# graphdeco-inria/editable-gaussian-reflections

Hardware: AMD Instinct MI355X
Metric: Mrays/s fwd+bwd @1080p, 1M Gaussians (higher is better)
Workload: dtype f32; 1 GPU; BASELINE config C: synthetic dense-init room+spheres cloud, HEADLINE variant = init (literal dense-init opacity 0.1 (config.py:44): Kc ~ 22 per ray, bounces mostly die), N=1000000, 1920x1080, one training iteration: export + update_bvh + forward + backward + grad import, num_bounces=2, jitter on, reference default config; variant=init, gaussians=1000000, width=1920, height=1080, parallelism=image tiles x1 + 1 all-reduce of the launch's [22N] gradients, team_help=product default (on)

## Files before the change

### editable-gaussian-reflections_amd/csrc/forward_task.inc

```
        const uint32_t task = tq;
        const TaskGeom tg = task_geom(v, tb, lane);
        const StateRef S = state_of(v, task, lane);
        const size_t chain_head = (size_t)step * (BATCH ? v.num_tasks * v.batch_frames : v.num_tasks) + task;
        if (GRADS && lane == 0) v.task_last_block[chain_head] = 0xFFFFFFFFu;
        if constexpr (OBJ) {
            for (uint32_t j = 0; j < oq.num_bits; j++) oacc[j * EGR_WAVE + (uint32_t)lane] = 0.0f;
        }

        bool active = tg.inside;
        f3 ro = mk3(0, 0, 0), rd = mk3(0, 0, 1);
        uint32_t seed = 0;
        if (step == 0) {
            if (active) {
                if constexpr (BATCH) {
                    seed = tea4(tg.pixel_id, (uint32_t)*v.meta.total_num_calls + bframe + 1u);
                    ro = mk3(bcam[0], bcam[1], bcam[2]);
                    rd = primary_direction(v, tg.px, tg.py, *v.cfg.jitter_primary_rays != 0, seed, bcam[12], bcam + 3);
                } else {
                    seed = tea4(tg.pixel_id, (uint32_t)*v.meta.total_num_calls);
                    ro = mk3(v.cam.origin[0], v.cam.origin[1], v.cam.origin[2]);
                    rd = primary_direction(v, tg.px, tg.py, *v.cfg.jitter_primary_rays != 0, seed, tanf(*v.cam.vertical_fov_radians / 2.0f), v.cam.rotation_w2c);
                }
            }
        } else {
// ... 22 lines not shown
            return e < v.ext_blocks_cap ? e : EGR_EXT_NONE - 1u;
        };
        double full_Td = 1.0;
        float full_T = 1.0f;
        bool overflow = false;
        EGR_STATS(uint32_t st_visits = 0, st_leafhits = 0, st_inner = 0, st_outer = 0, st_batches = 0u; unsigned long long st_eval_cycles = 0ull, st_batch_cycles = 0ull;)
        int seg = 0;
        float seg_lo, seg_hi;
        auto evaluate = [&](uint32_t prim, const float4 &w0, const float4 &w1, const float4 &w2, auto a2src, const f3 &lo_pre) {
            float t = 0.0f, alpha = 0.0f;
            const int r = test_candidate<CUBE, false>(fc, step, seg, near_plane, ro, rd, prim, w0, w1, w2, a2src, t, alpha, &lo_pre);
            if (r == 0 || r == 3) return;
            traversed++;
            if (r == 1) return;
            full_Td *= 1.0 - (double)alpha;
            if (cnt < v.cand_cap) {
                keys[EGR_KEY_AT(lane, cnt)] = t;
                vals[EGR_VAL_AT(lane, cnt)] = make_float2(alpha, u2f(prim));
                cnt++;
            } else {
                if (ext == EGR_EXT_NONE) ext = ext_alloc();
                const uint32_t e = cnt - v.cand_cap;
                if (ext < EGR_EXT_NONE - 1u && e < EGR_EXT_BLOCK) {
                    v.ext_keys[(size_t)ext * EGR_EXT_BLOCK + e] = t;
                    v.ext_vals[(size_t)ext * EGR_EXT_BLOCK + e] = make_float2(alpha, u2f(prim));
                    cnt++;
                } else {
                    overflow = true;
                }
            }
        };
        const bool packet = step == 0 && v.rays_per_task == (uint32_t)EGR_WAVE;
        const bool by_pairs = !packet;
        if (by_pairs) {
            rayp[lane][0] = make_float4(ro.x, ro.y, ro.z, rd.x), rayp[lane][1] = make_float4(rd.y, rd.z, invq.x, invq.y), rayp[lane][2] = make_float4(invq.z, ncq.x, ncq.y, ncq.z);
            gcnt[lane] = 0u, gtrav[lane] = 0u, gext[lane] = EGR_EXT_NONE;
        }
        bool beyond_far_empty = false;
        if (!sentinels) {
            const float fx0 = v.frame.ox - 2.0f / v.frame.sx, fx1 = v.frame.ox + 65534.0f / v.frame.sx;
            const float fy0 = v.frame.oy - 2.0f / v.frame.sy, fy1 = v.frame.oy + 65534.0f / v.frame.sy;
            const float fz0 = v.frame.oz - 2.0f / v.frame.sz, fz1 = v.frame.oz + 65534.0f / v.frame.sz;
            const float dx = fmaxf(fabsf(ro.x - fx0), fabsf(ro.x - fx1)), dy = fmaxf(fabsf(ro.y - fy0), fabsf(ro.y - fy1)),
                        dz = fmaxf(fabsf(ro.z - fz0), fabsf(ro.z - fz1));
            const bool reaches = !(dx * dx + dy * dy + dz * dz < far_plane * far_plane * 0.999f);
            beyond_far_empty = __ballot(ray_ok && reaches) == 0ull;
        }
        const float near_c = near_plane, far_c = far_plane;
        seg_lo = near_c, seg_hi = far_c;
        for (seg = 0; seg < (CUBE ? 1 : 3); seg++) {
            if (seg == 1) {
                if (!(near_plane > 0.0f)) continue;
                seg_lo = 0.0f, seg_hi = near_c;
            } else if (seg == 2) {
                if (beyond_far_empty) continue;
                seg_lo = far_c, seg_hi = 3.0e38f;
            }
        if (packet) {
            const unsigned long long okm = __ballot(ray_ok);
            if (okm != 0ull) {
                auto wsum = [](float x) {
#pragma unroll
                    for (int off = 32; off > 0; off >>= 1) x += __shfl_xor(x, off);
                    return x;
                };
                auto wmin = [](float x) {
#pragma unroll
                    for (int off = 32; off > 0; off >>= 1) x = fminf(x, __shfl_xor(x, off));
                    return x;
                };
                auto wmax = [](float x) {
#pragma unroll
                    for (int off = 32; off > 0; off >>= 1) x = fmaxf(x, __shfl_xor(x, off));
                    return x;
                };
                auto uni = [](float x) { return u2f((uint32_t)__builtin_amdgcn_readfirstlane((int)f2u(x))); };
                const f3 dz = ray_ok ? rd : mk3(0, 0, 0);
                const f3 ew = normalize(mk3(wsum(dz.x), wsum(dz.y), wsum(dz.z)));
                const f3 eu = normalize(cross(fabsf(ew.z) < 0.9f ? mk3(0, 0, 1) : mk3(1, 0, 0), ew)), ev = cross(ew, eu);
                const float pw = dot(rd, ew), pu = dot(rd, eu) / pw, pv = dot(rd, ev) / pw;
                const bool narrow = wmin(ray_ok ? pw : 1.0f) > 0.5f && isfinite(ew.x + ew.y + ew.z);
                const float big = 3.0e38f, lat = 4e-6f;
                const float umin = narrow ? fminf(wmin(ray_ok ? pu : big) - lat, -lat) : -big, umax = narrow ? fmaxf(wmax(ray_ok ? pu : -big) + lat, lat) : big;
                const float vmin = narrow ? fminf(wmin(ray_ok ? pv : big) - lat, -lat) : -big, vmax = narrow ? fmaxf(wmax(ray_ok ? pv : -big) + lat, lat) : big;
                const float kappa = narrow ? wmax(ray_ok ? 1.0f / pw : 1.0f) * 1.000001f : big;
                const float isx = 1.0f / v.frame.sx, isy = 1.0f / v.frame.sy, isz = 1.0f / v.frame.sz;
                const f3 cam_o = BATCH ? mk3(bcam[0], bcam[1], bcam[2]) : mk3(v.cam.origin[0], v.cam.origin[1], v.cam.origin[2]);
                const float oqx = (cam_o.x - v.frame.ox) * v.frame.sx + 2.0f, oqy = (cam_o.y - v.frame.oy) * v.frame.sy + 2.0f, oqz = (cam_o.z - v.frame.oz) * v.frame.sz + 2.0f;
                const float hux = uni(0.5f * eu.x * isx), huy = uni(0.5f * eu.y * isy), huz = uni(0.5f * eu.z * isz);
                const float hvx = uni(0.5f * ev.x * isx), hvy = uni(0.5f * ev.y * isy), hvz = uni(0.5f * ev.z * isz);
                const float hwx = uni(0.5f * ew.x * isx), hwy = uni(0.5f * ew.y * isy), hwz = uni(0.5f * ew.z * isz);
                const float cu = uni(2.0f * (hux * oqx + huy * oqy + huz * oqz)), cv = uni(2.0f * (hvx * oqx + hvy * oqy + hvz * oqz)), cw = uni(2.0f * (hwx * oqx + hwy * oqy + hwz * oqz));
                const float slack = uni(isx + isy + isz);
                const float f_umin = uni(umin), f_umax = uni(umax), f_vmin = uni(vmin), f_vmax = uni(vmax), f_kappa = uni(kappa);
                const float f_lo = uni(seg_lo), f_hi = uni(seg_hi);
                const bool narrow_u = __builtin_amdgcn_readfirstlane(narrow ? 1 : 0) != 0;
                auto frustum_hit = [&](const uint4 &q) -> bool {
                    const float lx = (float)(q.x & 0xFFFFu), ly = (float)(q.x >> 16), lz = (float)(q.y & 0xFFFFu);
                    const float hx = (float)(q.y >> 16), hy = (float)(q.z & 0xFFFFu), hz = (float)(q.z >> 16);
                    const float cx = lx + hx, cy = ly + hy, cz = lz + hz, ex = hx - lx, ey = hy - ly, ez = hz - lz;
                    const float u1 = fmaf(hux, cx, fmaf(huy, cy, fmaf(huz, cz, -cu))), u2 = fmaf(fabsf(hux), ex, fmaf(fabsf(huy), ey, fabsf(huz) * ez));
                    const float v1 = fmaf(hvx, cx, fmaf(hvy, cy, fmaf(hvz, cz, -cv))), v2 = fmaf(fabsf(hvx), ex, fmaf(fabsf(hvy), ey, fabsf(hvz) * ez));
                    const float w1 = fmaf(hwx, cx, fmaf(hwy, cy, fmaf(hwz, cz, -cw))), w2 = fmaf(fabsf(hwx), ex, fmaf(fabsf(hwy), ey, fabsf(hwz) * ez));
                    const float wmx = w1 + w2 + slack, wmn = w1 - w2 - slack;
                    bool keep = wmx > 0.0f;
                    if (!narrow_u) return true;
                    keep &= fmaf(-f_umin, wmx, u1 + u2) >= -slack;
                    keep &= fmaf(f_umax, wmx, u2 - u1) >= -slack;
                    keep &= fmaf(-f_vmin, wmx, v1 + v2) >= -slack;
                    keep &= fmaf(f_vmax, wmx, v2 - v1) >= -slack;
                    keep &= wmx * f_kappa >= f_lo;
                    keep &= wmn <= f_hi;
                    if (sentinels) keep |= ((q.x & 0xFFFFu) == 0u) | ((q.x >> 16) == 0u) | ((q.y & 0xFFFFu) == 0u) | ((q.y >> 16) == 65535u) | ((q.z & 0xFFFFu) == 65535u) | ((q.z >> 16) == 65535u);
                    return keep;
                };
                const float n_umin = sqrtf(fmaf(f_umin, f_umin, 1.0f)), n_umax = sqrtf(fmaf(f_umax, f_umax, 1.0f)), n_vmin = sqrtf(fmaf(f_vmin, f_vmin, 1.0f)), n_vmax = sqrtf(fmaf(f_vmax, f_vmax, 1.0f));
                const uint32_t m = (uint32_t)lane & 7u, grp = (uint32_t)lane >> 3;
                uint32_t *__restrict__ ugstk = v.stack_spill + (size_t)slot * EGR_GSTK * EGR_WAVE;
                constexpr uint32_t UGSTK_CAP = (uint32_t)EGR_GSTK * EGR_WAVE;
                bool f_over = false;
                uint32_t top = 1u, nl = 0u;
                if (lane == 0) pstk[0] = 0u;
                wave_sync();
                for (;;) {
                    const bool do_eval = nl >= (uint32_t)EGR_WAVE || (top == 0u && nl > 0u);
                    if (!do_eval && top == 0u) break;
                    if (do_eval) {
                        EGR_STATS(const unsigned long long te0 = __builtin_amdgcn_s_memtime();)
                        if (narrow_u) {
                            EGR_STATS(const unsigned long long tf0 = __builtin_amdgcn_s_memtime(); st_batches += nl;)
                            uint32_t nk = 0u;
                            for (uint32_t base = 0u; base < nl; base += (uint32_t)EGR_WAVE) {
                                const uint32_t nb = min(nl - base, (uint32_t)EGR_WAVE);
                                const uint32_t leaf = lbuf[base + min((uint32_t)lane, nb - 1u)];
                                const float4 sp = v.bsph[leaf];
                                const f3 a = mk3(sp.x - cam_o.x, sp.y - cam_o.y, sp.z - cam_o.z);
                                const float au = dot(a, eu), av = dot(a, ev), aw = dot(a, ew);
                                const float rad = sqrtf(fmaxf(sp.w, 0.0f)) * 1.005f + 2e-6f * (fabsf(a.x) + fabsf(a.y) + fabsf(a.z));
                                bool keep = (uint32_t)lane < nb && sp.w >= 0.0f;
                                keep = keep && !(fmaf(f_umin, aw, -au) > rad * n_umin) && !(fmaf(-f_umax, aw, au) > rad * n_umax);
                                keep = keep && !(fmaf(f_vmin, aw, -av) > rad * n_vmin) && !(fmaf(-f_vmax, aw, av) > rad * n_vmax);
                                wave_sync();
                                const unsigned long long km = __builtin_amdgcn_ballot_w64(keep);
                                if (keep) lbuf[nk + __builtin_amdgcn_mbcnt_hi((uint32_t)(km >> 32), __builtin_amdgcn_mbcnt_lo((uint32_t)km, 0u))] = leaf;
                                nk += (uint32_t)__popcll(km);
                                wave_sync();
                            }
                            nl = nk;
                            EGR_STATS(st_batch_cycles += __builtin_amdgcn_s_memtime() - tf0;)
                        }
                        EGR_TIMES_IS(9, chain_leaves += nl;)
                        if (nl != 0u) {
                        static_assert(EGR_WAVE + 8 * EGR_FPOP * EGR_WIDTH <= 3 * EGR_WAVE, "the ray table holds one float4 per buffered leaf");
                        float4 *const llo = &rayp[0][0];
                        for (uint32_t base = 0u; base < nl; base += (uint32_t)EGR_WAVE) {
                            const uint32_t li = base + (uint32_t)lane;
                            if (li < nl) {
                                const uint32_t leaf = lbuf[li];
                                const float4 g0 = v.inst_w[4 * (size_t)leaf], g1 = v.inst_w[4 * (size_t)leaf + 1], g2 = v.inst_w[4 * (size_t)leaf + 2];
                                const f3 lo_ = object_origin(g0, g1, g2, cam_o);
                                llo[li] = make_float4(lo_.x, lo_.y, lo_.z, 0.0f);
                            }
                        }
                        wave_sync();
                        uint32_t pn = (uint32_t)__builtin_amdgcn_readfirstlane((int)lbuf[0]);
                        float4 n0 = load_f4_uniform(v.inst_w, 4 * pn), n1 = load_f4_uniform(v.inst_w, 4 * pn + 1), n2 = load_f4_uniform(v.inst_w, 4 * pn + 2), n3 = load_f4_uniform(v.inst_w, 4 * pn + 3);
                        uint32_t pn_next = lbuf[min(1u, nl - 1u)];
                        float4 nlo = llo[0];
#pragma unroll 1
                        for (uint32_t i = 0; i < nl; i++) {
                            const uint32_t p = pn;
                            const float4 w0 = n0, w1 = n1, w2 = n2, a2 = n3;
                            const f3 lo_pre = mk3(nlo.x, nlo.y, nlo.z);
                            pn = (uint32_t)__builtin_amdgcn_readfirstlane((int)pn_next);
                            pn_next = lbuf[min(i + 2u, nl - 1u)];
                            n0 = load_f4_uniform(v.inst_w, 4 * pn), n1 = load_f4_uniform(v.inst_w, 4 * pn + 1), n2 = load_f4_uniform(v.inst_w, 4 * pn + 2), n3 = load_f4_uniform(v.inst_w, 4 * pn + 3);
                            nlo = llo[min(i + 1u, nl - 1u)];
                            EGR_STATS(st_leafhits += ray_ok ? 1u : 0u, st_outer += (lane == 0);)
                            if (ray_ok) evaluate(p, w0, w1, w2, a2, lo_pre);
#if defined(__HIP_DEVICE_COMPILE__)
                            asm volatile("" ::"s"(n0.w), "s"(n1.w), "s"(n2.w), "s"(n3.x), "s"(n3.y));
#endif
                        }
                        }
                        nl = 0u;
                        wave_sync();
                        EGR_STATS(st_eval_cycles += __builtin_amdgcn_s_memtime() - te0;)
                        if (top == 0u) break;
                    }
                    const uint32_t npop = min(top, 8u * (uint32_t)EGR_FPOP);
                    uint4 sl_[EGR_FPOP];
#pragma unroll
                    for (int u = 0; u < EGR_FPOP; u++) {
                        const uint32_t gi = grp + 8u * (uint32_t)u;
                        const uint32_t e = top - 1u - min(gi, top - 1u);
                        uint32_t node = pstk[min(e, (uint32_t)EGR_PSTK - 1u)];
                        if (top > (uint32_t)EGR_PSTK && e >= (uint32_t)EGR_PSTK) node = __hip_atomic_load(ugstk + (e - EGR_PSTK), __ATOMIC_RELAXED, __HIP_MEMORY_SCOPE_AGENT);
                        sl_[u] = wnodes[(size_t)node * EGR_WIDTH + m];
                        if (!(gi < npop)) sl_[u].w = EGR_EMPTY_SLOT;
                        EGR_STATS(st_visits += (m == 0u && gi < npop) ? 1u : 0u;)
                    }
                    top -= npop;
                    EGR_STATS(st_inner += (lane == 0);)
                    wave_sync();
#pragma unroll
                    for (int u = 0; u < EGR_FPOP; u++) {
                        const uint4 sl = sl_[u];
                        const bool hit = frustum_hit(sl) & (sl.w != EGR_EMPTY_SLOT);
                        const bool leaf = (int)sl.w < 0;
                        const unsigned long long hm = __builtin_amdgcn_ballot_w64(hit), lm = __builtin_amdgcn_ballot_w64(leaf);
                        const unsigned long long im = hm & ~lm, fm = hm & lm;
                        const uint32_t at = top + __builtin_amdgcn_mbcnt_hi((uint32_t)(im >> 32), __builtin_amdgcn_mbcnt_lo((uint32_t)im, 0u));
                        if (hit & !leaf) {
                            if (at < (uint32_t)EGR_PSTK) pstk[at] = sl.w;
                            else if (at - EGR_PSTK < UGSTK_CAP) __hip_atomic_store(ugstk + (at - EGR_PSTK), sl.w, __ATOMIC_RELAXED, __HIP_MEMORY_SCOPE_AGENT);
                            else f_over = true;
                        }
                        top = min(top + (uint32_t)__popcll(im), (uint32_t)EGR_PSTK + UGSTK_CAP);
                        if (hit & leaf) lbuf[nl + __builtin_amdgcn_mbcnt_hi((uint32_t)(fm >> 32), __builtin_amdgcn_mbcnt_lo((uint32_t)fm, 0u))] = sl.w & ~EGR_LEAF_FLAG;
                        nl += (uint32_t)__popcll(fm);
                    }
                    wave_sync();
                }
                if (__ballot(f_over) != 0ull) overflow = true;
            }
        } else {
            const size_t scratch0 = (size_t)slot * EGR_WAVE;
            uint32_t *__restrict__ gstk = v.stack_spill + (size_t)slot * EGR_GSTK * EGR_WAVE;
            bool g_over = false;
            const uint32_t top = (uint32_t)__popcll(act_mask);
            if ((act_mask >> lane) & 1ull) pstk[__popcll(act_mask & ((1ull << lane) - 1ull))] = (uint32_t)lane << 26;
            if constexpr (TEAM > 1) {
                while (uniform_u32(lds_peek(&team.box_count[wv])) != 0u) __builtin_amdgcn_s_sleep(1);
                if (lane == 0) lds_poke(&team.ctx[wv][0], (uint32_t)step | ((uint32_t)seg << 8)), lds_poke(&team.ctx[wv][1], f2u(seg_lo)), lds_poke(&team.ctx[wv][2], f2u(seg_hi)), lds_poke(&team.ctx[wv][3], f2u(near_plane)), lds_poke(&team.ctx[wv][4], (uint32_t)wv);
            }
            wave_sync();
            WalkStats wst;
            if (!sentinels && seg == 0) pair_walk<false, true, CUBE, TEAM>(v, fc, wsh, wsh, team, wv, scratch0, gstk, step, seg, seg_lo, seg_hi, near_plane, top, g_over, wst);
            else if (sentinels) pair_walk<true, false, CUBE, TEAM>(v, fc, wsh, wsh, team, wv, scratch0, gstk, step, seg, seg_lo, seg_hi, near_plane, top, g_over, wst);
            else pair_walk<false, false, CUBE, TEAM>(v, fc, wsh, wsh, team, wv, scratch0, gstk, step, seg, seg_lo, seg_hi, near_plane, top, g_over, wst);
            EGR_TIMES(tt_batches += wst.inner, tt_evals += wst.outer, tt_offers += wst.offers, tt_tall += wst.tall;)
            EGR_STATS(st_visits += wst.visits, st_leafhits += wst.leafhits, st_inner += wst.inner, st_outer += wst.outer;)
            EGR_STATS(if (lane == 0 && (wst.offers | wst.tall)) atomicAdd(v.control + DG_TEAM_OFFERS, wst.offers), atomicAdd(v.control + DG_TEAM_TALL, wst.tall);)
            if (TEAM > 1 && v.team_help) {
                EGR_TIMES(const unsigned long long tw0 = __builtin_amdgcn_s_memrealtime();)
                team_help_while<CUBE, TEAM>(v, fc, wsh_all, team, wv, blockIdx.x * (uint32_t)TEAM, g_over, [&]() { return uniform_u32(lds_peek(&team.busy[wv])) != 0u; });
                EGR_TIMES(tt_wait += __builtin_amdgcn_s_memrealtime() - tw0;)
                __builtin_amdgcn_fence(__ATOMIC_ACQUIRE, "workgroup");
            }
            if (__ballot(g_over) != 0ull) overflow = true;
        }

        }
        if (by_pairs) {
            ext = gext[lane], traversed = gtrav[lane];
            cnt = min(gcnt[lane], v.cand_cap + (ext < EGR_EXT_NONE - 1u ? EGR_EXT_BLOCK : 0u));
            if (cnt != gcnt[lane]) overflow = true;
            const uint32_t nbase = min(cnt, v.cand_cap);
            for (uint32_t k = 0; k < nbase; k += 8) {
                const float4 a = EGR_VAL_Q(lane, k), b = EGR_VAL_Q(lane, k + 2), c = EGR_VAL_Q(lane, k + 4), d = EGR_VAL_Q(lane, k + 6);
                const float al[8] = {a.x, a.z, b.x, b.z, c.x, c.z, d.x, d.z};
#pragma unroll
                for (int j = 0; j < 8; j++)
                    if (k + (uint32_t)j < nbase) full_Td *= 1.0 - (double)al[j];
            }
            for (uint32_t k = nbase; k < cnt; k++) full_Td *= 1.0 - (double)v.ext_vals[(size_t)ext * EGR_EXT_BLOCK + (k - v.cand_cap)].x;
        }
        full_T = (float)full_Td;
#ifdef EGR_DEBUG_PIXEL
        if (active && step == 0 && tg.pixel_id == (uint32_t)EGR_DEBUG_PIXEL) {
            printf("[pixel %u] cnt %u traversed %u full_T %.9g\n", tg.pixel_id, cnt, traversed, (double)full_T);
            for (uint32_t k = 0; k < cnt && k < v.cand_cap; k++) printf("   k %u t %.9g (%08x) alpha %.9g pos %u gid %u\n", k, (double)keys[EGR_KEY_AT(lane, k)], f2u(keys[EGR_KEY_AT(lane, k)]), (double)vals[EGR_VAL_AT(lane, k)].x, f2u(vals[EGR_VAL_AT(lane, k)].y), v.gid_of_pos[f2u(vals[EGR_VAL_AT(lane, k)].y)]);
        }
#endif
#ifdef EGR_DEBUG_LIST
        if (active && cnt > 0 && cnt <= v.cand_cap) {
            double p = 1.0;
            for (uint32_t k = 0; k < cnt; k++) p *= 1.0 - (double)vals[EGR_VAL_AT(lane, k)].x;
            if (fabs(p - (double)full_T) > 1e-4 * fmax(p, (double)full_T) + 1e-12) {
                printf("[list mismatch] step %d task %u lane %d cnt %u prodlist %.9g full_T %.9g pair walk %d\n", step, task, lane, cnt, p, (double)full_T, (int)by_pairs);
                for (uint32_t k = 0; k < cnt && k < 40; k++) printf("   k %u t %.9g alpha %.9g pos %u\n", k, (double)keys[EGR_KEY_AT(lane, k)], (double)vals[EGR_VAL_AT(lane, k)].x, f2u(vals[k].y));
            }
        }
#endif
        EGR_STATS(const unsigned long long tm1 = __builtin_amdgcn_s_memtime(); {
            const uint32_t cm = wave_max_u32(active ? cnt : 0u);
            const unsigned long long a = wave_sum_u32(st_visits), b = wave_sum_u32(st_leafhits), c2 = wave_sum_u32(st_inner), d = wave_sum_u32(st_outer);
            if (lane == 0 && step == 0) atomicAdd(v.control + DG_LIST_HIST + (cm <= 16u ? 0 : cm <= 24u ? 1 : cm <= 32u ? 2 : cm <= 40u ? 3 : cm <= 48u ? 4 : cm <= 64u ? 5 : 6), 1u);
            if (lane == 0 && st_batches) atomicAdd(diag64(v.control, DG_FILTER_CYC), st_batch_cycles), atomicAdd(diag64(v.control, DG_FILTER_LEAVES), (unsigned long long)st_batches);
            if (lane == 0) atomicAdd(diag64(v.control, DG_LEAF_EVAL_CYC, step > 0), st_eval_cycles), atomicAdd(diag64(v.control, DG_VISITS, step > 0), a), atomicAdd(diag64(v.control, DG_LEAF_HITS, step > 0), b), atomicAdd(diag64(v.control, DG_WALK_ITERS, step > 0), c2), atomicAdd(diag64(v.control, DG_EVAL_ROUNDS, step > 0), d);
        })
        EGR_TIMES(const unsigned long long tt_mid = __builtin_amdgcn_s_memrealtime();)
        f3 c_rgb = mk3(0, 0, 0), c_n = mk3(0, 0, 0), c_f0 = mk3(0, 0, 0);
        float c_rough = 0.0f, c_depth = 0.0f, T = 1.0f;
        uint32_t nhits = 0;
        {
            float t_prev = near_plane;
            uint32_t k_prev = 0xFFFFFFFFu;
            bool running = active && cnt > 0;
            uint32_t last_block = 0xFFFFFFFFu, cur_block = 0xFFFFFFFFu;
            bool recording = GRADS;
            EGR_STATS(unsigned long long tc_scan = 0ull, tc_alloc = 0ull, tc_av = 0ull, tc_p1 = 0ull, tc_app = 0ull;)
            for (uint32_t it = 0;; it += EGR_HIT_BLOCK_ROWS) {
                EGR_STATS(const unsigned long long tcs0 = __builtin_amdgcn_s_memtime();)
                float kt[8];
                uint32_t ki[8];
#pragma unroll
                for (int j = 0; j < 8; j++) kt[j] = 3.4028235e38f, ki[j] = 0xFFFFFFFFu;
                if ((it & 15u) == 0u) k_prev = 0xFFFFFFFFu;
                if (running) {
                    auto consider = [&](float tk, uint32_t k) {
                        if (!(tk >= t_prev && tk < kt[7])) return;
                        if (tk == t_prev && !(k > k_prev && k_prev != 0xFFFFFFFFu)) return;
                        const float x = tk;
                        const bool c0 = x < kt[0], c1 = x < kt[1], c2 = x < kt[2], c3 = x < kt[3], c4 = x < kt[4], c5 = x < kt[5], c6 = x < kt[6], c7 = x < kt[7];
                        ki[7] = c6 ? ki[6] : (c7 ? k : ki[7]), kt[7] = __builtin_amdgcn_fmed3f(x, kt[6], kt[7]);
                        ki[6] = c5 ? ki[5] : (c6 ? k : ki[6]), kt[6] = __builtin_amdgcn_fmed3f(x, kt[5], kt[6]);
                        ki[5] = c4 ? ki[4] : (c5 ? k : ki[5]), kt[5] = __builtin_amdgcn_fmed3f(x, kt[4], kt[5]);
                        ki[4] = c3 ? ki[3] : (c4 ? k : ki[4]), kt[4] = __builtin_amdgcn_fmed3f(x, kt[3], kt[4]);
                        ki[3] = c2 ? ki[2] : (c3 ? k : ki[3]), kt[3] = __builtin_amdgcn_fmed3f(x, kt[2], kt[3]);
                        ki[2] = c1 ? ki[1] : (c2 ? k : ki[2]), kt[2] = __builtin_amdgcn_fmed3f(x, kt[1], kt[2]);
                        ki[1] = c0 ? ki[0] : (c1 ? k : ki[1]), kt[1] = __builtin_amdgcn_fmed3f(x, kt[0], kt[1]);
                        ki[0] = c0 ? k : ki[0], kt[0] = fminf(x, kt[0]);
                    };
                    const uint32_t nbase = min(cnt, v.cand_cap);
                    uint32_t k = 0;
                    for (; k + 16 <= nbase; k += 16) {
                        const float4 ka = EGR_KEY_Q(lane, k), kb = EGR_KEY_Q(lane, k + 4);
                        const float4 kc = EGR_KEY_Q(lane, k + 8), kd = EGR_KEY_Q(lane, k + 12);
                        consider(ka.x, k), consider(ka.y, k + 1), consider(ka.z, k + 2), consider(ka.w, k + 3);
                        consider(kb.x, k + 4), consider(kb.y, k + 5), consider(kb.z, k + 6), consider(kb.w, k + 7);
                        consider(kc.x, k + 8), consider(kc.y, k + 9), consider(kc.z, k + 10), consider(kc.w, k + 11);
                        consider(kd.x, k + 12), consider(kd.y, k + 13), consider(kd.z, k + 14), consider(kd.w, k + 15);
                    }
                    if (k + 8 <= nbase) {
// ... 165 lines not shown
```

### editable-gaussian-reflections_amd/csrc/trace.hip

```cpp
#include <algorithm>
#include <cstdio>
#include <cstdlib>
#include <type_traits>
#include <utility>
#include <vector>

#define EGR_CONTRACT_AFTER_EPILOGUE
#include "egr_diag.hpp"
#include "egr_epilogue.hpp"

#ifndef EGR_GPOP
#define EGR_GPOP 5
#endif
#define EGR_WALK_MAX_LEAVES (8 * EGR_GPOP * EGR_WIDTH)
#define EGR_LBUF (64 + 2 * EGR_WALK_MAX_LEAVES)
#ifndef EGR_FPOP
#define EGR_FPOP 2
#endif
#ifndef EGR_PSTK
#define EGR_PSTK 512
#endif

namespace {

// ... 142 lines not shown
    return base[idx];
#endif
}
EGR_DI bool slab_clip(float ax, float bx, float ay, float by, float az, float bz, float tmin, float tmax) {
    const float t0 = fmaxf(fmaxf(fminf(ax, bx), fminf(ay, by)), fmaxf(fminf(az, bz), tmin));
    const float t1 = fminf(fminf(fmaxf(ax, bx), fmaxf(ay, by)), fminf(fmaxf(az, bz), tmax));
    return t0 <= t1;
}
EGR_DI bool qslab_hit(uint4 q, f3 invq, f3 ncq, float tmin, float tmax) {
    const uint32_t lx = q.x & 0xFFFFu, ly = q.x >> 16, lz = q.y & 0xFFFFu, hx = q.y >> 16, hy = q.z & 0xFFFFu, hz = q.z >> 16;
    const float flx = lx == 0u ? -3.0e38f : (float)lx, fly = ly == 0u ? -3.0e38f : (float)ly, flz = lz == 0u ? -3.0e38f : (float)lz;
    const float fhx = hx == 65535u ? 3.0e38f : (float)hx, fhy = hy == 65535u ? 3.0e38f : (float)hy, fhz = hz == 65535u ? 3.0e38f : (float)hz;
    const float ax = fmaf(flx, invq.x, ncq.x), bx = fmaf(fhx, invq.x, ncq.x);
    const float ay = fmaf(fly, invq.y, ncq.y), by = fmaf(fhy, invq.y, ncq.y);
    const float az = fmaf(flz, invq.z, ncq.z), bz = fmaf(fhz, invq.z, ncq.z);
    return slab_clip(ax, bx, ay, by, az, bz, tmin, tmax);
}
EGR_DI bool qslab_hit_inframe(uint4 q, f3 invq, f3 ncq, float tmin, float tmax) {
    const float flx = (float)(q.x & 0xFFFFu), fly = (float)(q.x >> 16), flz = (float)(q.y & 0xFFFFu);
    const float fhx = (float)(q.y >> 16), fhy = (float)(q.z & 0xFFFFu), fhz = (float)(q.z >> 16);
    const float ax = fmaf(flx, invq.x, ncq.x), bx = fmaf(fhx, invq.x, ncq.x);
    const float ay = fmaf(fly, invq.y, ncq.y), by = fmaf(fhy, invq.y, ncq.y);
    const float az = fmaf(flz, invq.z, ncq.z), bz = fmaf(fhz, invq.z, ncq.z);
    return slab_clip(ax, bx, ay, by, az, bz, tmin, tmax);
}
EGR_DI float4 fetch_a2(const float4 *p) { return *p; }
EGR_DI float4 fetch_a2(float4 v) { return v; }
EGR_DI bool hits_unit_cube(f3 lo, f3 ld, float tmin, float tmax) {
    f3 inv = mk3(__builtin_amdgcn_rcpf(ld.x), __builtin_amdgcn_rcpf(ld.y), __builtin_amdgcn_rcpf(ld.z));
    float t0 = tmin, t1 = tmax;
    bool ok = true;
#define EGR_AXIS(c)                                                            \
    if (ld.c != 0.0f) {                                                        \
        float a = (-1.0f - lo.c) * inv.c, b = (1.0f - lo.c) * inv.c;           \
        t0 = fmaxf(t0, fminf(a, b));                                           \
        t1 = fminf(t1, fmaxf(a, b));                                           \
    } else if (lo.c < -1.0f || lo.c > 1.0f)                                    \
        ok = false;
    EGR_AXIS(x) EGR_AXIS(y) EGR_AXIS(z)
#undef EGR_AXIS
    return ok && t0 <= t1;
}

EGR_DI bool hits_unit_cube_exact(f3 lo, f3 ld, float tmin, float tmax) {
    float t0 = tmin, t1 = tmax;
    bool ok = true;
#define EGR_AXIS(c)                                                            \
    if (ld.c != 0.0f) {                                                        \
        float a = (-1.0f - lo.c) / ld.c, b = (1.0f - lo.c) / ld.c;             \
        t0 = fmaxf(t0, fminf(a, b));                                           \
        t1 = fminf(t1, fmaxf(a, b));                                           \
    } else if (lo.c < -1.0f || lo.c > 1.0f)                                    \
        ok = false;
    EGR_AXIS(x) EGR_AXIS(y) EGR_AXIS(z)
#undef EGR_AXIS
    return ok && t0 <= t1;
}

#ifndef EGR_TEAM
#define EGR_TEAM 16
#endif
#ifndef EGR_BOX
#define EGR_BOX 128
#endif
#ifndef EGR_DONATE_MIN
#define EGR_DONATE_MIN 96
#endif
#define EGR_BOX_CLAIMED 0x80000000u
#define EGR_EXT_LOCKED (EGR_EXT_NONE - 2u)

EGR_DI void wave_sync() {
    __builtin_amdgcn_fence(__ATOMIC_RELEASE, "wavefront");
    __builtin_amdgcn_wave_barrier();
    __builtin_amdgcn_fence(__ATOMIC_ACQUIRE, "wavefront");
}
typedef __attribute__((address_space(3))) uint32_t egr_lds_u32;
EGR_DI uint32_t lds_peek(const uint32_t *p) { return *(const volatile egr_lds_u32 *)p; }
EGR_DI void lds_poke(uint32_t *p, uint32_t x) { *(volatile egr_lds_u32 *)p = x; }
EGR_DI uint32_t uniform_u32(uint32_t x) { return (uint32_t)__builtin_amdgcn_readfirstlane((int)x); }

struct FwdConst {
    float exp_power, transmittance_threshold, backfacing_max_dist, backfacing_thr, far_plane;
    int num_bounces;
    bool sentinels;
    const float4 *__restrict__ app;
    const uint4 *__restrict__ wnodes;
};
struct ObjectQuery {
    const uint32_t *pos_bits;
    uint32_t num_bits;
    float *masks;
    uint32_t *hit;
    int32_t *top;
};
struct ObjectBitList {
    uint8_t bit[32];
};
struct WalkShared {
    uint32_t pstk[EGR_PSTK];
    uint32_t lbuf[EGR_LBUF];
    float4 rayp[EGR_WAVE][3];
    uint32_t gcnt[EGR_WAVE], gtrav[EGR_WAVE];
    uint32_t gext[EGR_WAVE];
    uint32_t wc[4 * EGR_NSTEPS];
};
template <int TEAM> struct TeamShared {
    uint32_t done;
    uint32_t hungry;
    uint32_t box_count[TEAM];
    uint32_t busy[TEAM];
    uint32_t ctx[TEAM][5];
    uint32_t box[TEAM][EGR_BOX];
};
struct WalkStats {
    uint32_t visits = 0, leafhits = 0, inner = 0, outer = 0;
    uint32_t offers = 0, tall = 0;
};

template <bool CUBE, bool SEG0, class A2>
EGR_DI int test_candidate(const FwdConst &fc, int step, int seg, float near_plane, const f3 &o, const f3 &d, uint32_t prim, const float4 &w0, const float4 &w1,
                          const float4 &w2, A2 a2src, float &t, float &alpha, const f3 *lo_pre = nullptr) {
    const float far_plane = fc.far_plane;
    f3 lo, ld, dhat, u;
    bool behind, outside;
    if (lo_pre != nullptr) {
        lo = *lo_pre;
        candidate_geometry_from(w0, w1, w2, lo, d, ld, dhat, t, u, behind, outside);
    } else {
        candidate_geometry(w0, w1, w2, o, d, lo, ld, dhat, t, u, behind, outside);
    }
    if constexpr (CUBE) {
        if (!hits_unit_cube_exact(lo, ld, near_plane, far_plane)) return 0;
    } else {
        if constexpr (SEG0) {
            if (!(t >= near_plane && t <= far_plane)) return 0;
        } else if (!(seg == 0 ? (t >= near_plane && t <= far_plane) : seg == 1 ? (t < near_plane) : (t > far_plane))) return 0;
        if constexpr (!SEG0)
            if (seg != 0 && !hits_unit_cube(lo, ld, near_plane, far_plane)) return 0;
    }
    if (outside) return CUBE ? 1 : 3;
    if (behind) return 1;
    if (step != 0 && t < fc.backfacing_max_dist) {
        const float4 n0 = fc.app[2 * prim], n1 = fc.app[2 * prim + 1];
        f3 gn = mk3(n0.w, n1.x, n1.y);
        if (sqrtf(egr_dot3(gn.x, gn.y, gn.z, gn.x, gn.y, gn.z)) > fc.backfacing_thr && egr_dot3(gn.x, gn.y, gn.z, dhat.x, dhat.y, dhat.z) > 0.0f) return 1;
    }
    const float4 a2 = fetch_a2(a2src);
    f3 x = u * a2.w;
    float gaussval = egr_gaussian_sq(egr_dot3(x.x, x.y, x.z, x.x, x.y, x.z), fc.exp_power);
    alpha = EGR_MAX_ALPHA * gaussval * a2.z;
    return 2;
}

template <bool CUBE, bool SEG0>
EGR_DI void pair_eval_append(const DeviceView &v, const FwdConst &fc, WalkShared &rays, const size_t scratch0, const int step, const int seg, const float near_plane, const bool have,
                             const uint32_t er, const uint32_t pidx, const float4 &w0, const float4 &w1, const float4 &w2, const float4 &w3, bool &g_over, WalkStats &st) {
    const int lane = threadIdx.x & (EGR_WAVE - 1);
    (void)lane;
    int res = 0;
    float t = 0.0f, alpha = 0.0f;
    if (have) {
        const float4 q0 = rays.rayp[er][0], q1 = rays.rayp[er][1];
        res = test_candidate<CUBE, SEG0>(fc, step, seg, near_plane, mk3(q0.x, q0.y, q0.z), mk3(q0.w, q1.x, q1.y), pidx, w0, w1, w2, w3, t, alpha);
    }
    EGR_WALK(st.leafhits += have ? 1u : 0u; st.outer += (lane == 0);)
    if (res == 1 || res == 2) atomicAdd(&rays.gtrav[er], 1u);
    uint32_t at = 0u;
    if (res == 2) at = atomicAdd(&rays.gcnt[er], 1u);
    const bool in_ext = res == 2 && at >= v.cand_cap;
    if (res == 2 && !in_ext) {
        const size_t slot = (scratch0 + er) * v.cand_cap + at;
        v.cand_keys[scratch0 * v.cand_cap + ((((size_t)(at >> 2) * EGR_WAVE + er) << 2) + (at & 3u))] = t;
        v.cand_vals[slot] = make_float2(alpha, u2f(pidx));
    }
    if (__ballot(in_ext) != 0ull) {
        for (;;) {
            const unsigned long long pend = __ballot(in_ext && lds_peek(&rays.gext[er]) == EGR_EXT_NONE);
            if (pend == 0ull) break;
            const int src = __ffsll((long long)pend) - 1;
            if (lane == src && atomicCAS(&rays.gext[er], EGR_EXT_NONE, EGR_EXT_LOCKED) == EGR_EXT_NONE) {
                const uint32_t e = atomicAdd(v.control + CW_EXT_BUMP, 1u);
                lds_poke(&rays.gext[er], e < v.ext_blocks_cap ? e : EGR_EXT_NONE - 1u);
            }
            wave_sync();
        }
        if (in_ext) {
            uint32_t e = lds_peek(&rays.gext[er]);
            while (e == EGR_EXT_LOCKED) __builtin_amdgcn_s_sleep(1), e = lds_peek(&rays.gext[er]);
            const uint32_t k = at - v.cand_cap;
            if (e < EGR_EXT_NONE - 1u && k < EGR_EXT_BLOCK) {
                v.ext_keys[(size_t)e * EGR_EXT_BLOCK + k] = t;
                v.ext_vals[(size_t)e * EGR_EXT_BLOCK + k] = make_float2(alpha, u2f(pidx));
            } else {
                g_over = true;
            }
        }
    }
}

template <bool SENT, bool SEG0, bool CUBE, int TEAM>
EGR_DI void pair_walk(const DeviceView &v, const FwdConst &fc, WalkShared &mine, WalkShared &rays, TeamShared<TEAM> &team, const int self, const size_t scratch0,
                      uint32_t *__restrict__ gstk, const int step, const int seg, const float seg_lo, const float seg_hi, const float near_plane, uint32_t top,
                      bool &g_over, WalkStats &st) {
    const int lane = threadIdx.x & (EGR_WAVE - 1);
    const uint32_t m = (uint32_t)lane & 7u, grp = (uint32_t)lane >> 3;
    constexpr uint32_t GSTK_CAP = (uint32_t)EGR_GSTK * EGR_WAVE;
    const uint4 *__restrict__ wnodes = fc.wnodes;
    uint32_t nl = 0u;
    uint32_t hungry_seen = 0u;
    for (;;) {
        const bool do_eval = nl >= (uint32_t)EGR_WAVE || (top == 0u && nl > 0u);
        if (!do_eval && top == 0u) {
            if constexpr (TEAM > 1) {
                uint32_t r = 0u;
                if (lane == 0) {
                    const uint32_t c = lds_peek(&team.box_count[self]);
                    if (c != 0u && !(c & EGR_BOX_CLAIMED) && atomicCAS(&team.box_count[self], c, c | EGR_BOX_CLAIMED) == c) r = c;
                }
                r = uniform_u32(r);
                if (r != 0u) {
                    r &= 0xFFFFu;
                    for (uint32_t i = (uint32_t)lane; i < r; i += EGR_WAVE) mine.pstk[i] = team.box[self][i];
                    top = r;
                    wave_sync();
                    if (lane == 0) lds_poke(&team.box_count[self], 0u);
                    continue;
                }
            }
            break;
        }
        bool have = false;
        uint32_t er = 0u, pidx = 0u;
        float4 w0 = make_float4(0, 0, 0, 0), w1 = w0, w2 = w0, w3 = w0;
        if (do_eval) {
            const uint32_t take = min(nl, (uint32_t)EGR_WAVE);
            nl -= take;
            have = (uint32_t)lane < take;
            const uint32_t pr = mine.lbuf[nl + min((uint32_t)lane, take - 1u)];
            er = pr >> 26, pidx = pr & 0x03FFFFFFu;
            if (have) w0 = v.inst_w[4 * pidx], w1 = v.inst_w[4 * pidx + 1], w2 = v.inst_w[4 * pidx + 2], w3 = v.inst_w[4 * pidx + 3];
        }
        const uint32_t npop = nl + (uint32_t)EGR_WALK_MAX_LEAVES <= (uint32_t)EGR_LBUF ? min(top, 8u * (uint32_t)EGR_GPOP) : 0u;
        uint32_t pw[EGR_GPOP];
        uint4 sl_[EGR_GPOP];
        if constexpr (TEAM > 1) hungry_seen = lds_peek(&team.hungry);
        if (npop != 0u) {
#pragma unroll
            for (int u = 0; u < EGR_GPOP; u++) pw[u] = mine.pstk[min(top - 1u - min(grp + 8u * (uint32_t)u, top - 1u), (uint32_t)EGR_PSTK - 1u)];
            if (top > (uint32_t)EGR_PSTK) {
#pragma unroll
                for (int u = 0; u < EGR_GPOP; u++) {
                    const uint32_t e = top - 1u - min(grp + 8u * (uint32_t)u, top - 1u);
                    if (grp + 8u * (uint32_t)u < npop && e >= (uint32_t)EGR_PSTK) pw[u] = *reinterpret_cast<const volatile uint32_t *>(gstk + (e - EGR_PSTK));
                }
            }
#pragma unroll
            for (int u = 0; u < EGR_GPOP; u++) {
                sl_[u] = wnodes[(size_t)(pw[u] & 0x03FFFFFFu) * EGR_WIDTH + m];
                if (!(grp + 8u * (uint32_t)u < npop)) sl_[u].w = EGR_EMPTY_SLOT;
            }
            top -= npop;
            EGR_WALK(st.visits += (m == 0u) ? min(npop > grp ? (npop - grp + 7u) / 8u : 0u, (uint32_t)EGR_GPOP) : 0u; st.inner += (lane == 0);)
        }
        wave_sync();
        if (do_eval) pair_eval_append<CUBE, SEG0>(v, fc, rays, scratch0, step, seg, near_plane, have, er, pidx, w0, w1, w2, w3, g_over, st);
        if (npop != 0u) {
#pragma unroll
            for (int u = 0; u < EGR_GPOP; u++) {
                const uint32_t rtag = pw[u] & 0xFC000000u;
                const float4 q1 = rays.rayp[pw[u] >> 26][1], q2 = rays.rayp[pw[u] >> 26][2];
                const uint4 sl = sl_[u];
                const bool hit = (SENT ? qslab_hit(sl, mk3(q1.z, q1.w, q2.x), mk3(q2.y, q2.z, q2.w), seg_lo, seg_hi) : qslab_hit_inframe(sl, mk3(q1.z, q1.w, q2.x), mk3(q2.y, q2.z, q2.w), seg_lo, seg_hi)) & (sl.w != EGR_EMPTY_SLOT);
                const bool leaf = (int)sl.w < 0;
                const unsigned long long hm = __builtin_amdgcn_ballot_w64(hit), lm = __builtin_amdgcn_ballot_w64(leaf);
                const unsigned long long im = hm & ~lm, fm = hm & lm;
                const uint32_t at = top + __builtin_amdgcn_mbcnt_hi((uint32_t)(im >> 32), __builtin_amdgcn_mbcnt_lo((uint32_t)im, 0u));
                if (top + (uint32_t)EGR_WAVE <= (uint32_t)EGR_PSTK) {
                    if (hit & !leaf) mine.pstk[at] = rtag | sl.w;
                    top += (uint32_t)__popcll(im);
                } else {
                    if (hit & !leaf) {
                        if (at < (uint32_t)EGR_PSTK) mine.pstk[at] = rtag | sl.w;
                        else if (at - EGR_PSTK < GSTK_CAP) gstk[at - EGR_PSTK] = rtag | sl.w;
                        else g_over = true;
                    }
                    top = min(top + (uint32_t)__popcll(im), (uint32_t)EGR_PSTK + GSTK_CAP);
                }
                if (hit & leaf) mine.lbuf[nl + __builtin_amdgcn_mbcnt_hi((uint32_t)(fm >> 32), __builtin_amdgcn_mbcnt_lo((uint32_t)fm, 0u))] = rtag | (sl.w & ~EGR_LEAF_FLAG);
                nl += (uint32_t)__popcll(fm);
            }
        }
        wave_sync();
        EGR_WALK(st.tall += (lane == 0 && top >= (uint32_t)EGR_DONATE_MIN) ? 1u : 0u;)
        if constexpr (TEAM > 1) {
            if (uniform_u32(hungry_seen) != 0u && top >= (uint32_t)EGR_DONATE_MIN && top <= (uint32_t)EGR_PSTK && uniform_u32(lds_peek(&team.box_count[self])) == 0u) {
                const uint32_t give = min(top >> 1, (uint32_t)EGR_BOX);
                for (uint32_t base = 0u; base < top; base += EGR_WAVE) {
                    const uint32_t i = base + (uint32_t)lane;
                    const uint32_t x = mine.pstk[min(i, (uint32_t)EGR_PSTK - 1u)];
                    wave_sync();
                    if (i < 2u * give) {
                        if (i & 1u) team.box[self][i >> 1] = x;
                        else mine.pstk[i >> 1] = x;
                    } else if (i < top) mine.pstk[i - give] = x;
                }
                top -= give;
// ... 1202 lines not shown
```

Before: 472.8 Mrays/s.

## Cull buffered leaves per ray with bounding-sphere test and compact per-lane eval lists

For the non-cube path, each 64-leaf chunk stages leaf transforms, opacity data and a normalized bounding-sphere center in LDS. Each lane then tests every staged leaf against its own ray with a conservative cross-product sphere test and builds a bitmask. Lanes step through only their own surviving leaves instead of evaluating every leaf uniformly. This avoids full Gaussian evaluation for leaves the ray clearly misses, at the cost of extra LDS staging, a per-lane O(64) sphere loop, and divergent per-lane leaf order, which loses the scalar uniform loads.

```diff
diff --git a/editable-gaussian-reflections_amd/csrc/forward_task.inc b/editable-gaussian-reflections_amd/csrc/forward_task.inc
--- a/editable-gaussian-reflections_amd/csrc/forward_task.inc
+++ b/editable-gaussian-reflections_amd/csrc/forward_task.inc
@@ -198,6 +198,8 @@
                         EGR_TIMES_IS(9, chain_leaves += nl;)
                         if (nl != 0u) {
                         static_assert(EGR_WAVE + 8 * EGR_FPOP * EGR_WIDTH <= 3 * EGR_WAVE, "the ray table holds one float4 per buffered leaf");
+                        static_assert(3 * EGR_WAVE + 5 * EGR_WAVE <= EGR_LBUF, "the leaf buffer holds five more words per leaf of a 64-leaf chunk behind its 192 leaf indices");
+                        if constexpr (CUBE) {
                         float4 *const llo = &rayp[0][0];
                         for (uint32_t base = 0u; base < nl; base += (uint32_t)EGR_WAVE) {
                             const uint32_t li = base + (uint32_t)lane;
@@ -227,6 +229,70 @@
 #if defined(__HIP_DEVICE_COMPILE__)
                             asm volatile("" ::"s"(n0.w), "s"(n1.w), "s"(n2.w), "s"(n3.x), "s"(n3.y));
 #endif
+                        }
+                        } else {
+                        constexpr int NW = EGR_WAVE / 32;
+                        uint32_t *const lx = lbuf + 3 * EGR_WAVE;
+                        const float rd2 = dot(rd, rd);
+                        for (uint32_t cbase = 0u; cbase < nl; cbase += (uint32_t)EGR_WAVE) {
+                        const uint32_t cn = min(nl - cbase, (uint32_t)EGR_WAVE);
+                        if ((uint32_t)lane < cn) {
+                            const uint32_t leaf = lbuf[cbase + (uint32_t)lane];
+                            const float4 g0 = v.inst_w[4 * (size_t)leaf], g1 = v.inst_w[4 * (size_t)leaf + 1], g2 = v.inst_w[4 * (size_t)leaf + 2], g3 = v.inst_w[4 * (size_t)leaf + 3];
+                            const f3 lo_ = object_origin(g0, g1, g2, cam_o);
+                            const f3 an = staged_sphere(v.bsph[leaf], g0, g1, g2, lo_, cam_o);
+                            rayp[lane][0] = make_float4(g0.x, g0.y, g0.z, lo_.x), rayp[lane][1] = make_float4(g1.x, g1.y, g1.z, lo_.y), rayp[lane][2] = make_float4(g2.x, g2.y, g2.z, lo_.z);
+                            lx[5 * lane] = f2u(g3.z), lx[5 * lane + 1] = f2u(g3.w), lx[5 * lane + 2] = f2u(an.x), lx[5 * lane + 3] = f2u(an.y), lx[5 * lane + 4] = f2u(an.z);
+                        }
+                        wave_sync();
+                        uint32_t mk[NW];
+#pragma unroll
+                        for (int w = 0; w < NW; w++) {
+                            uint32_t m = 0u;
+                            if (32u * (uint32_t)w < cn) {
+                                const uint32_t nb = min(cn - 32u * (uint32_t)w, 32u);
+#pragma unroll 4
+                                for (uint32_t j = 0; j < nb; j++) {
+                                    const uint32_t i = 32u * (uint32_t)w + j;
+                                    const f3 an = mk3(u2f(lx[5u * i + 2u]), u2f(lx[5u * i + 3u]), u2f(lx[5u * i + 4u]));
+                                    m |= (ray_misses_sphere(an, rd, rd2) ? 0u : 1u) << j;
+                                }
+                            }
+                            mk[w] = ray_ok ? m : 0u;
+                        }
+                        constexpr uint32_t NO_SLOT = 0xFFFFFFFFu;
+                        auto pop = [&]() -> uint32_t {
+                            uint32_t word = 0u, base = 0u;
+#pragma unroll
+                            for (int w = NW - 1; w >= 0; w--) {
+                                const bool h = mk[w] != 0u;
+                                word = h ? mk[w] : word, base = h ? 32u * (uint32_t)w : base;
+                            }
+                            const uint32_t rest = word & (word - 1u);
+#pragma unroll
+                            for (int w = 0; w < NW; w++) mk[w] = base == 32u * (uint32_t)w ? rest : mk[w];
+                            return base + (uint32_t)__ffs((int)word) - 1u;
+                        };
+                        uint32_t s_n = pop();
+                        uint32_t sc = min(s_n, cn - 1u);
+                        uint32_t leaf_n = lbuf[cbase + sc];
+                        float4 n0 = rayp[sc][0], n1 = rayp[sc][1], n2 = rayp[sc][2];
+                        float q0 = u2f(lx[5u * sc]), q1 = u2f(lx[5u * sc + 1u]);
+#pragma unroll 1
+                        while (__ballot(s_n != NO_SLOT) != 0ull) {
+                            const bool have = s_n != NO_SLOT;
+                            const uint32_t p = leaf_n;
+                            const float4 w0 = n0, w1 = n1, w2 = n2, a2 = make_float4(0.0f, 0.0f, q0, q1);
+                            const f3 lo_pre = mk3(n0.w, n1.w, n2.w);
+                            s_n = pop(), sc = min(s_n, cn - 1u);
+                            leaf_n = lbuf[cbase + sc];
+                            n0 = rayp[sc][0], n1 = rayp[sc][1], n2 = rayp[sc][2];
+                            q0 = u2f(lx[5u * sc]), q1 = u2f(lx[5u * sc + 1u]);
+                            EGR_STATS(st_leafhits += have ? 1u : 0u, st_outer += (lane == 0);)
+                            if (have) evaluate(p, w0, w1, w2, a2, lo_pre);
+                        }
+                        wave_sync();
+                        }
                         }
                         }
                         nl = 0u;
diff --git a/editable-gaussian-reflections_amd/csrc/trace.hip b/editable-gaussian-reflections_amd/csrc/trace.hip
--- a/editable-gaussian-reflections_amd/csrc/trace.hip
+++ b/editable-gaussian-reflections_amd/csrc/trace.hip
@@ -318,6 +318,23 @@
     return 2;
 }
 
+EGR_DI f3 staged_sphere(const float4 &sp, const float4 &w0, const float4 &w1, const float4 &w2, const f3 &lo, const f3 &o) {
+    const f3 a = mk3(sp.x - o.x, sp.y - o.y, sp.z - o.z);
+    const float smax = sqrtf(fmaxf(sp.w, 0.0f));
+    const float inv_smin = sqrtf(fmaxf(fmaxf(dot(mk3(w0.x, w0.y, w0.z), mk3(w0.x, w0.y, w0.z)), dot(mk3(w1.x, w1.y, w1.z), mk3(w1.x, w1.y, w1.z))),
+                                       dot(mk3(w2.x, w2.y, w2.z), mk3(w2.x, w2.y, w2.z))));
+    const float lo1 = fabsf(lo.x) + fabsf(lo.y) + fabsf(lo.z);
+    const float rad = smax * (1.005f + 1e-6f * lo1 * (smax * inv_smin + 1.0f)) + 2e-6f * (fabsf(a.x) + fabsf(a.y) + fabsf(a.z)) +
+                      1e-6f * (fabsf(o.x) + fabsf(o.y) + fabsf(o.z) + fabsf(sp.x) + fabsf(sp.y) + fabsf(sp.z));
+    const float ir = sp.w >= 0.0f ? 1.0f / rad : u2f(0x7FC00000u);
+    return mk3(a.x * ir, a.y * ir, a.z * ir);
+}
+EGR_DI bool ray_misses_sphere(const f3 &an, const f3 &d, float d2) {
+    const f3 c = cross(an, d);
+    const float c2 = dot(c, c);
+    return c2 > d2 && c2 < __builtin_inff();
+}
+
 template <bool CUBE, bool SEG0>
 EGR_DI void pair_eval_append(const DeviceView &v, const FwdConst &fc, WalkShared &rays, const size_t scratch0, const int step, const int seg, const float near_plane, const bool have,
                              const uint32_t er, const uint32_t pidx, const float4 &w0, const float4 &w1, const float4 &w2, const float4 &w3, bool &g_over, WalkStats &st) {
```

Measured after the change: 478.2 Mrays/s (median of 6 runs). +1.1%, better.
